# Iselix/kwiiyatta

Measured on AMD Instinct MI355X. Metric: frames/sec end-to-end analyse->align->convert->synth, 48 kHz 5 ms hop, higher is better.
Workload: dtype f64; 1 GPU; config3: 48 kHz source (10 s, T=2001) + target (11 s, T=2201) pairs: CheapTrick+D4C of both, pad with freshly drawn silent spectra, sp2mc, FastDTW(radius 32) align, GMM(64 comp, D=144)+MLPG convert, mc2sp, WORLD synthesis; pairs_per_gpu=32, streams_per_gpu=4, GPU_MAX_HW_QUEUES=4, launch=the whole step is one captured HIP graph, gmm_model_prepared=once per converter (the per-mixture matrices depend on the GMM only), parallelism=pairs in lockstep x32 per GPU, pair-per-GPU x1, no collective

## Files before the change

### kwiiyatta_amd/csrc/kwy_synth.hip

```cpp
#include <math.h>
#include <stdlib.h>

#include <algorithm>
#include <vector>

#include "kwy_internal.hpp"

#define SYN_DEFAULT_F0 500.0
#define SYN_TILE_PER_THREAD 4
#define SYN_TILE (KWY_THREADS * SYN_TILE_PER_THREAD)
#define SYN_TWO_PI (2.0 * KWY_PI)
#define SYN_SLOTS(y_length, fs) ((int)((y_length) * 640 / (fs)) + 64)

struct syn_params {
  int64_t T, y_length;
  int fs, fft_size;
  double frame_period;
  double lowest_f0;
  double sp_mul;
};

__device__ __forceinline__ double syn_increment(const double *__restrict__ f0, const syn_params &p,
                                                int64_t n, double *vuv_out) {
  const double fp = p.frame_period;
// ... 459 lines not shown
          int i = tid * SYN_PH_PER_THREAD + j;
          if (i >= pos && i < cross) {
            if (direct) wrap[tile0 + i] = fmod(ldexp((double)mv[j], k - 52), SYN_TWO_PI);
            if (i == cross - 1) s_tp = ldexp((double)mv[j], k - 52);
          }
        }
        if (cross > pos && !direct) {
          if (tid == 0) { segs[tix].start[nseg] = pos; segs[tix].end[nseg] = cross; segs[tix].tp[nseg] = tp; }
          ++nseg;
        }
        __syncthreads();
        if (cross > pos) tp = s_tp;
      }
      if (cross < tile_n && tp == 0.0) {
        const int nw = min(SYN_WARM, tile_n - cross);
        if (tid < nw) s_c[tid] = inc[tile0 + cross + tid];
        __syncthreads();
        if (tid == 0) {
          double t = 0.0;
          int q = 0;
          for (; q + 8 <= nw; q += 8) {
            double v[8];
#pragma unroll
            for (int u = 0; u < 8; ++u) v[u] = s_c[q + u];
#pragma unroll
            for (int u = 0; u < 8; ++u) { t = t + v[u]; v[u] = t; }
#pragma unroll
            for (int u = 0; u < 8; ++u) s_tps[q + u] = v[u];
          }
          for (; q < nw; ++q) { t = t + s_c[q]; s_tps[q] = t; }
          s_tp = t;
        }
        __syncthreads();
        if (tid < nw) wrap[tile0 + cross + tid] = fmod(s_tps[tid], SYN_TWO_PI);
        tp = s_tp;
        pos = cross + nw;
      } else if (cross < tile_n) {
        tp = tp + inc[tile0 + cross];
        if (tid == 0) wrap[tile0 + cross] = fmod(tp, SYN_TWO_PI);
        pos = cross + 1;
      } else {
        pos = tile_n;
      }
      __syncthreads();
      ++n_rounds;
    }
    if (tid == 0) segs[tix].n = nseg;
    ++tix;
    SYN_DBG_SLOW();
  }
  if (dbg && tid == 0) {
    dbg[40] = clock64() - t_begin; dbg[41] = wall_clock64() - w_begin; dbg[42] = t_fast; dbg[43] = t_slow;
    dbg[44] = n_fast; dbg[45] = n_slow; dbg[46] = n_rounds;
  }
}

__device__ __forceinline__ void syn_tile_apply_body(const double *__restrict__ inc, int64_t y_length,
                                                               const double *__restrict__ tin,
                                                               const syn_segs *__restrict__ segs,
                                                               double *__restrict__ wrap) {
  __shared__ syn_ff wtot[2 * KWY_WAVES + 1];
  const int t = blockIdx.x, tid = threadIdx.x;
  const double tp_tile = tin[t];
  const bool fast = tp_tile > 0.0;
  const int ns = fast ? 1 : segs[t].n;
  const int64_t base = (int64_t)t * SYN_PH_TILE + (int64_t)tid * SYN_TL_PER_THREAD;
  double c[SYN_TL_PER_THREAD];
#pragma unroll
  for (int j = 0; j < SYN_TL_PER_THREAD; ++j) c[j] = (base + j < y_length) ? inc[base + j] : 0.0;
  double tpv[SYN_TL_PER_THREAD];
#pragma unroll
  for (int j = 0; j < SYN_TL_PER_THREAD; ++j) tpv[j] = -1.0;
  for (int q = 0; q < ns; ++q) {
    const double tp = fast ? tp_tile : segs[t].tp[q];
    const int s0 = fast ? 0 : segs[t].start[q], s1 = fast ? SYN_PH_TILE : segs[t].end[q];
    const int k = syn_exponent(tp);
    const unsigned long long tb = (unsigned long long)__double_as_longlong(tp);
    const long long m_in = (long long)((tb & 0xfffffffffffffULL) | 0x10000000000000ULL);
    const bool active = ((tid | 63) + 1) * SYN_TL_PER_THREAD > s0 && (tid & ~63) * SYN_TL_PER_THREAD < s1;
    syn_ff f[SYN_TL_PER_THREAD];
    syn_ff mine = {0, 0};
    if (active) {
#pragma unroll
      for (int j = 0; j < SYN_TL_PER_THREAD; ++j) {
        const int li = tid * SYN_TL_PER_THREAD + j;
        f[j] = (li >= s0 && li < s1 && base + j < y_length) ? syn_ff_make(c[j], k) : syn_ff{0, 0};
        mine = syn_ff_compose(mine, f[j]);
      }
    }
    syn_ff all;
    const syn_ff excl = syn_ff_block_exscan<KWY_WAVES>(mine, wtot, &all);
    if (active) {
      long long m = m_in + ((m_in & 1) ? excl.d1 : excl.d0);
#pragma unroll
      for (int j = 0; j < SYN_TL_PER_THREAD; ++j) {
        const int li = tid * SYN_TL_PER_THREAD + j;
        if (li >= s0 && li < s1 && base + j < y_length) {
          m += (m & 1) ? f[j].d1 : f[j].d0;
          tpv[j] = ldexp((double)m, k - 52);
        }
      }
    }
    __syncthreads();
  }
#pragma unroll
  for (int j = 0; j < SYN_TL_PER_THREAD; ++j)
    if (tpv[j] >= 0.0) wrap[base + j] = fmod(tpv[j], SYN_TWO_PI);
}

__device__ __forceinline__ bool syn_is_pulse(const double *__restrict__ wrap, int64_t n, int64_t y_length) {
  return n < y_length - 1 && fabs(wrap[n + 1] - wrap[n]) > KWY_PI;
}

__device__ __forceinline__ void syn_pulse_count_body(const double *__restrict__ wrap,
                                                                int64_t y_length, int *__restrict__ cnt) {
  __shared__ int sh[KWY_WAVES];
  const int64_t base = (int64_t)blockIdx.x * SYN_TILE + (int64_t)threadIdx.x * SYN_TILE_PER_THREAD;
  int c = 0;
#pragma unroll
  for (int j = 0; j < SYN_TILE_PER_THREAD; ++j) c += syn_is_pulse(wrap, base + j, y_length) ? 1 : 0;
  int tot;
  (void)kwy_block_exscan(c, sh, &tot);
  if (threadIdx.x == 0) cnt[blockIdx.x] = tot;
}

__device__ __forceinline__ void syn_pulse_emit_body(const double *__restrict__ wrap,
                                                               int64_t y_length, int fs,
                                                               const int *__restrict__ tile_off,
                                                               int cap, int32_t *__restrict__ pidx,
                                                               double *__restrict__ pshift) {
  __shared__ int sh[KWY_WAVES];
  const int64_t base = (int64_t)blockIdx.x * SYN_TILE + (int64_t)threadIdx.x * SYN_TILE_PER_THREAD;
  int c = 0;
#pragma unroll
  for (int j = 0; j < SYN_TILE_PER_THREAD; ++j) c += syn_is_pulse(wrap, base + j, y_length) ? 1 : 0;
  int tot;
  int pos = tile_off[blockIdx.x] + kwy_block_exscan(c, sh, &tot);
#pragma unroll
  for (int j = 0; j < SYN_TILE_PER_THREAD; ++j) {
    int64_t n = base + j;
    if (syn_is_pulse(wrap, n, y_length)) {
      if (pos < cap) {
        double y1 = wrap[n] - SYN_TWO_PI;
        double y2 = wrap[n + 1];
        double xx = -y1 / (y2 - y1);
        pidx[pos] = (int32_t)n;
        pshift[pos] = xx / fs;
      }
      ++pos;
    }
  }
}

struct syn_plan {
  int *npulse;
  int *tile_cnt;
  unsigned char *vuv8;
  int32_t *pidx;
  double *pshift;
};
struct syn_plan_view {
  const double *f0;
  syn_params p;
  syn_plan pl;
  double *incr, *wrap, *tsum, *tin;
  long long *summ;
  syn_segs *segs;
  syn_chunks *chunks;
  int cap;
};
struct syn_plan_batch {
  int n;
  long long *dbg;
  syn_plan_view u[KWY_BATCH_MAX];
};
__device__ __forceinline__ int syn_npt(int64_t y_length) { return (int)((y_length + SYN_PH_TILE - 1) / SYN_PH_TILE); }
__device__ __forceinline__ int syn_nt(int64_t y_length) { return (int)((y_length + SYN_TILE - 1) / SYN_TILE); }

__global__ __launch_bounds__(KWY_THREADS) void k_syn_inc(syn_plan_batch b) {
  const syn_plan_view &v = b.u[blockIdx.y];
  syn_inc_body(v.f0, v.p, v.incr, v.pl.vuv8);
}
__global__ __launch_bounds__(KWY_THREADS) void k_syn_tile_sums(syn_plan_batch b) {
  const syn_plan_view &v = b.u[blockIdx.y];
  if ((int)blockIdx.x >= syn_npt(v.p.y_length)) return;
  syn_tile_sums_body(v.incr, v.p.y_length, v.tsum);
}
__global__ __launch_bounds__(KWY_THREADS) void k_syn_tile_summary(syn_plan_batch b) {
  const syn_plan_view &v = b.u[blockIdx.y];
  const int npt = syn_npt(v.p.y_length);
  if ((int)blockIdx.x >= npt) return;
  syn_tile_summary_body(v.incr, v.p.y_length, v.tsum, npt, v.summ, v.chunks);
}
__global__ __launch_bounds__(SYN_PH_THREADS) void k_syn_phase(syn_plan_batch b) {
  const syn_plan_view &v = b.u[blockIdx.x];
  syn_phase_body(v.incr, v.p.y_length, v.summ, v.tin, v.segs, v.chunks, v.wrap, b.dbg);
}
__global__ __launch_bounds__(KWY_THREADS) void k_syn_tile_apply(syn_plan_batch b) {
  const syn_plan_view &v = b.u[blockIdx.y];
  if ((int)blockIdx.x >= syn_npt(v.p.y_length)) return;
  syn_tile_apply_body(v.incr, v.p.y_length, v.tin, v.segs, v.wrap);
}
__global__ __launch_bounds__(KWY_THREADS) void k_syn_pulse_count(syn_plan_batch b) {
  const syn_plan_view &v = b.u[blockIdx.y];
  if ((int)blockIdx.x >= syn_nt(v.p.y_length)) return;
  syn_pulse_count_body(v.wrap, v.p.y_length, v.pl.tile_cnt);
}
__global__ __launch_bounds__(KWY_THREADS) void k_syn_scan_counts(syn_plan_batch b) {
  const syn_plan_view &v = b.u[blockIdx.x];
  syn_scan_counts_body(v.pl.tile_cnt, syn_nt(v.p.y_length), v.pl.npulse);
}
__global__ __launch_bounds__(KWY_THREADS) void k_syn_pulse_emit(syn_plan_batch b) {
  const syn_plan_view &v = b.u[blockIdx.y];
  if ((int)blockIdx.x >= syn_nt(v.p.y_length)) return;
  syn_pulse_emit_body(v.wrap, v.p.y_length, v.p.fs, v.pl.tile_cnt, v.cap, v.pl.pidx, v.pl.pshift);
}

template <int LOG2N>
struct syn_pulse_nt { static constexpr int value = LOG2N <= 10 ? 64 : (LOG2N == 11 ? 128 : 256); };

template <int LOG2N>
struct syn_pulse_form {
  static constexpr bool SHORT = LOG2N == 11;
  static constexpr bool E_IN_BUF = SHORT, HALF_FIRST = SHORT, FUSED_FOLD = SHORT;
  static constexpr int H = 1 << (LOG2N - 1), TWL = (H / 8 > 1) ? H / 8 : 1;
  static constexpr size_t lds = sizeof(kwy_c) * ((H + 1) + TWL) + sizeof(double) * ((H + 2) + 8) +
                                (E_IN_BUF ? 0 : sizeof(uint32_t) * KWY_EBASE_WORDS);
};

template <int LOG2H, int NT, int V>
__device__ inline void syn_rfft_inplace(kwy_c *z, const kwy_c *__restrict__ tw, const kwy_c *__restrict__ pw, const kwy_c (&base)[V],
                                        const kwy_c *__restrict__ twN) {
  kwy_fft_inplace<LOG2H, NT, false>(z, tw, pw);
  kwy_syn_rsplit<LOG2H, NT, V>(z, base, twN);
}

template <int LOG2H, int NT, int V>
__device__ inline void syn_irfft_inplace(kwy_c *z, const kwy_c *__restrict__ tw, const kwy_c *__restrict__ pw, const kwy_c (&base)[V],
                                         const kwy_c *__restrict__ twN) {
  constexpr int H = 1 << LOG2H, N = 2 * H;
  constexpr bool TABLE = 8 * (NT * V) / N < 1;
  const int tid = kwy_tid_opaque();
  __syncthreads();
#pragma unroll
  for (int r = 0; r * NT <= H / 2; ++r) {
    const int k = tid + NT * r;
    if (k > H / 2) continue;
    if (k == 0) {
      const double ar = z[0].x, br = z[H].x;
      z[0] = {ar + br, ar - br};
    } else {
      kwy_c w;
      if constexpr (TABLE) w = twN[k]; else w = syn_pair_twiddle<LOG2H, NT, V>(base, r);
      const kwy_c A = z[k], Bc = z[H - k];
      const double er = A.x + Bc.x, ei = A.y - Bc.y;
      const double dr = A.x - Bc.x, di = A.y + Bc.y;
      const double wr = w.x, wi = -w.y;
      const double orr = __builtin_fma(dr, wr, -(di * wi)), oi = __builtin_fma(dr, wi, di * wr);
      z[k] = {er - oi, ei + orr};
      if (k != H - k) z[H - k] = {er + oi, -(ei - orr)};
    }
  }
  __syncthreads();
  kwy_fft_inplace<LOG2H, NT, true>(z, tw, pw);
}

template <int NT, int V>
__device__ __forceinline__ double syn_block_sum_v(const double (&part)[V], double *red) {
  double ws[V];
#pragma unroll
  for (int g = 0; g < V; ++g) ws[g] = kwy_wave_sum(part[g]);
  __syncthreads();
  if ((threadIdx.x & 63) == 0) {
#pragma unroll
    for (int g = 0; g < V; ++g) red[(threadIdx.x >> 6) + (NT / 64) * g] = ws[g];
  }
  __syncthreads();
  double s = red[0];
#pragma unroll
  for (int i = 1; i < NT * V / 64; ++i) s += red[i];
  return s;
}

__device__ __forceinline__ double syn_safe_ap(double x) {
  return fmax(0.001, fmin(0.999999999999, x));
}

struct syn_view {
  const double *sp, *ap;
  syn_params p;
  const int32_t *pidx;
  const double *pshift;
  const unsigned char *vuv8;
  const int *npulse, *tile_off;
  int cap, slots, nt;
  double *resp, *y;
};
typedef kwy_batch<syn_view> syn_batch;

template <int LOG2N, bool DIRECT>
__global__ __launch_bounds__(syn_pulse_nt<LOG2N>::value, LOG2N <= 11 ? 3 : (LOG2N == 12 ? 2 : 1)) void k_syn_pulse(
    syn_batch batch, kwy_randn_src rs, const uint4 *__restrict__ poly,
    const kwy_c *__restrict__ twH, const kwy_c *__restrict__ twP, const kwy_c *__restrict__ twN,
    const double *__restrict__ dc_remover, long long *__restrict__ dbg) {
  constexpr int NT = syn_pulse_nt<LOG2N>::value, V = KWY_THREADS / NT;
  bool stamping = false;
#define SYN_STAMP(n) do { if (stamping && threadIdx.x == 0) dbg[n] = clock64(); } while (0)
  const int utt = batch.find(blockIdx.x);
  const int lblock = (int)blockIdx.x - batch.start[utt], lgrid = batch.start[utt + 1] - batch.start[utt];
  const double *__restrict__ sp = batch.u[utt].sp, *__restrict__ ap = batch.u[utt].ap;
  const syn_params p = batch.u[utt].p;
  const int32_t *__restrict__ pidx = batch.u[utt].pidx;
  const double *__restrict__ pshift = batch.u[utt].pshift;
  const unsigned char *__restrict__ vuv8 = batch.u[utt].vuv8;
  const int *__restrict__ npulse = batch.u[utt].npulse;
  const int cap = batch.u[utt].cap;
  const int first_pulse = DIRECT ? batch.u[utt].slots : 0, slots = DIRECT ? cap : batch.u[utt].slots;
  double *__restrict__ resp = batch.u[utt].resp;
  double *__restrict__ y = batch.u[utt].y;
  constexpr int N = 1 << LOG2N, H = N / 2, K = H + 1;
  constexpr int C = N / NT;
  constexpr int RK = (H + 1 + NT - 1) / NT;
  constexpr int TWL = (H / 8 > 1) ? H / 8 : 1;
  typedef syn_pulse_form<LOG2N> F;
  extern __shared__ double smem[];
  double *red = smem;
  uint32_t *e_own = (uint32_t *)(red + 8);
  kwy_c *twl = (kwy_c *)(e_own + (F::E_IN_BUF ? 0 : KWY_EBASE_WORDS));
  kwy_c *buf = twl + TWL;
  double *lap = (double *)(buf + (H + 1));
  uint32_t *e = F::E_IN_BUF ? (uint32_t *)(buf + 512) : e_own;
  static_assert(!F::E_IN_BUF || sizeof(kwy_c) * (H + 1) >= 8192 + sizeof(uint32_t) * KWY_EBASE_WORDS, "no room");

  const int tid = threadIdx.x;
  for (int i = tid; i < TWL; i += NT) twl[i] = twH[i];
  kwy_c twb[V];
#pragma unroll
  for (int g = 0; g < V; ++g) twb[g] = twN[tid + NT * g];
  const int P = min(npulse[0], cap);
  const int pend = min(P, first_pulse + slots);
  for (int pp = first_pulse + lblock; pp < pend; pp += lgrid) {
    const int tid = kwy_tid_opaque();
    const int idx = pidx[pp];
    const int nxt = pidx[min(P - 1, pp + 1)];
    const int noise_size = nxt - idx;
    __syncthreads();
    if (noise_size <= 0) continue;
    const int ns_used = min(noise_size, N);
    const double current_vuv = vuv8[idx] ? 1.0 : 0.0;
    const double current_time = idx / (double)p.fs;
    const double shift = pshift[pp];

    int fl = (int)floor(current_time / p.frame_period);
    int ce = (int)ceil(current_time / p.frame_period);
    if (fl > p.T - 1) fl = (int)p.T - 1;
    if (ce > p.T - 1) ce = (int)p.T - 1;
    const double interpolation = current_time / p.frame_period - fl;
    const double *s0 = sp + (int64_t)fl * K, *s1 = sp + (int64_t)ce * K;
    const double *a0 = ap + (int64_t)fl * K, *a1 = ap + (int64_t)ce * K;
    double rv0 = syn_safe_ap(a0[0]);
    if (fl != ce) rv0 = (1.0 - interpolation) * rv0 + interpolation * syn_safe_ap(a1[0]);
    const bool has_periodic = current_vuv > 0.5 && !(rv0 * rv0 > 0.999);
    stamping = dbg && threadIdx.x == 0 && has_periodic && blockIdx.x >= (unsigned)dbg[63] && dbg[62] == 0 &&
               atomicCAS((unsigned long long *)&dbg[62], 0ull, 1ull) == 0ull;
    SYN_STAMP(0);
    {
      double *L = (double *)buf;
      double evs[RK], rts[RK];
#pragma unroll
      for (int r = 0; r < RK; ++r) {
        const int k = min(tid + NT * r, H);
        double ev, rv;
        if (fl == ce) {
          ev = fabs(s0[k] * p.sp_mul);
          rv = syn_safe_ap(a0[k]);
        } else {
          ev = (1.0 - interpolation) * fabs(s0[k] * p.sp_mul) + interpolation * fabs(s1[k] * p.sp_mul);
          rv = (1.0 - interpolation) * syn_safe_ap(a0[k]) + interpolation * syn_safe_ap(a1[k]);
        }
        evs[r] = ev;
        rts[r] = rv * rv;
      }
#pragma unroll
      for (int r = 0; r < RK; ++r) {
        const int k = tid + NT * r;
        if (k <= H) {
          lap[k] = kwy_log((current_vuv != 0.0) ? evs[r] * rts[r] : evs[r]) / 2.0;
          if (has_periodic) L[k] = kwy_log(evs[r] * (1.0 - rts[r]) + KWY_SAFE) / 2.0;
        }
      }
    }

    double dc_component = 0.0;
    SYN_STAMP(1);
#pragma nounroll
    for (int part = has_periodic ? 0 : 1; part < 2; ++part) {
      const int tid = kwy_tid_opaque();
      double *L = (double *)buf;
      if (part == 1) {
        double la[RK], wv[RK];
#pragma unroll
        for (int r = 0; r < RK; ++r) {
          const int k = tid + NT * r;
          la[r] = k <= H ? lap[k] : 0.0;
          wv[r] = (has_periodic && k < H) ? L[k] : 0.0;
        }
        __syncthreads();
#pragma unroll
        for (int r = 0; r < RK; ++r) {
          const int k = tid + NT * r;
          if (k <= H) { L[k] = la[r]; lap[k] = wv[r]; }
        }
      }
      kwy_c mp[RK];
#pragma unroll
      for (int r = 0; r < RK; ++r) mp[r] = {0.0, 0.0};
#pragma nounroll
      for (int it = 0; it < 2 + part; ++it) {
        const int tid = kwy_tid_opaque();
        bool dense_first = true;
        if (it == 0) {
          __syncthreads();
          for (int i = H + 1 + tid; i < N; i += NT) L[i] = L[N - i];
          __syncthreads();
        } else if (it == 1) {
          if constexpr (!F::FUSED_FOLD) kwy_syn_fold<LOG2N - 1, NT, !F::HALF_FIRST>(buf);
          if constexpr (F::HALF_FIRST) {
            kwy_fft_pass8_first_half_core<LOG2N - 1, NT, false>(buf, kwy_tw_table{twl});
            dense_first = false;
          }
        } else {
#pragma unroll
          for (int r = 0; r < RK; ++r) {
            const int k = tid + NT * r;
            mp[r] = k <= H ? buf[k] : kwy_c{0.0, 0.0};
          }
          __syncthreads();
          const uint64_t dpos = (uint64_t)(idx - pidx[0]);
          uint32_t raw[C];
          if (dpos + (uint64_t)ns_used <= rs.n) {
#pragma unroll
            for (int j = 0; j < C; ++j) raw[j] = (tid + NT * j < ns_used) ? rs.tab[dpos + tid + NT * j] : 0u;
          } else {
            kwy_rng_block_ebase(dpos, rs.pow2, e);
            kwy_rng rng;
            if constexpr (sizeof(kwy_c) * (H + 1) >= 8192) {
              kwy_rng_build_table<NT>(e, (uint4 *)buf);
              __syncthreads();
              rng = kwy_rng_combine_table((const uint4 *)buf, poly[tid]);
              __syncthreads();
            } else {
              rng = kwy_rng_combine(e, poly[tid]);
            }
            uint32_t *D = (uint32_t *)buf;
#pragma unroll
            for (int j = 0; j < C; ++j) D[C * tid + j] = kwy_rng_randn_raw(rng);
            __syncthreads();
#pragma unroll
            for (int j = 0; j < C; ++j) raw[j] = D[tid + NT * j];
            __syncthreads();
          }
          double nv[C];
          double sum[V];
#pragma unroll
          for (int g = 0; g < V; ++g) sum[g] = 0.0;
#pragma unroll
          for (int j = 0; j < C; ++j) {
            const int d = tid + NT * j;
            nv[j] = kwy_randn_from_raw(raw[j]);
            if (d < ns_used) sum[j % V] += nv[j];
          }
          const double average = syn_block_sum_v<NT, V>(sum, red) / noise_size;
#pragma unroll
          for (int j = 0; j < C; ++j) {
            const int d = tid + NT * j;
            L[d] = (d < ns_used) ? nv[j] - average : 0.0;
          }
          __syncthreads();
        }
        if constexpr (!F::SHORT) {
          syn_rfft_inplace<LOG2N - 1, NT, V>(buf, twl, twP, twb, twN);
        } else {
          if (dense_first) kwy_fft_pass8<LOG2N - 1, 0, NT, false>(buf, twl);
          kwy_fft_inplace_rest<LOG2N - 1, NT, false>(buf, twl, twP);
          if (F::FUSED_FOLD && it == 0) kwy_syn_rsplit_fold<LOG2N - 1, NT, V, !F::HALF_FIRST>(buf, twb, twN);
          else kwy_syn_rsplit<LOG2N - 1, NT, V>(buf, twb, twN);
        }
        if (it == 1) {
          constexpr int G = 3;
#pragma nounroll
          for (int k0 = tid; k0 <= H; k0 += G * NT) {
            kwy_c R[G];
#pragma unroll
            for (int g = 0; g < G; ++g) R[g] = buf[min(k0 + g * NT, H)];
#pragma unroll
            for (int g = 0; g < G; ++g) {
              const double tmp = exp(R[g].x / N);
              const double ph = R[g].y / N;
              double sn, cs;
              kwy_sincos_medium(ph, &sn, &cs);
              R[g] = {tmp * cs, tmp * sn};
            }
#pragma unroll
            for (int g = 0; g < G; ++g)
              if (k0 + g * NT <= H) buf[k0 + g * NT] = R[g];
          }
          __syncthreads();
        }
      }
      SYN_STAMP(2 + 5 * part);
      if (part == 0) {
        const double coefficient = 2.0 * KWY_PI * shift * p.fs / N;
        for (int k = tid; k <= H; k += NT) {
          const double re = buf[k].x, im = buf[k].y;
          const double re2 = kwy_cos_pi_range(coefficient * k);
          const double im2 = sqrt(1.0 - re2 * re2);
          buf[k] = {__builtin_fma(re, re2, im * im2), __builtin_fma(im, re2, -(re * im2))};
        }
      } else {
#pragma unroll
        for (int r = 0; r < RK; ++r) {
          const int k = tid + NT * r;
          if (k <= H) buf[k] = cmulf(mp[r], buf[k]);
        }
      }
      SYN_STAMP(3 + 5 * part);
      syn_irfft_inplace<LOG2N - 1, NT, V>(buf, twl, twP, twb, twN);
      SYN_STAMP(4 + 5 * part);
      if (part == 0) {
        const double *w = (const double *)buf;
        double ps[V];
#pragma unroll
        for (int g = 0; g < V; ++g) {
          ps[g] = 0.0;
          for (int i = tid + NT * g; i < H; i += KWY_THREADS) ps[g] += w[i];
        }
        dc_component = syn_block_sum_v<NT, V>(ps, red);
        SYN_STAMP(5);
      }
    }
    {
      const int tid = kwy_tid_opaque();
      SYN_STAMP(10);
      const double *w = (const double *)buf;
      const double sqrt_noise_size = sqrt((double)noise_size);
      double *slot = DIRECT ? nullptr : resp + (size_t)(pp - first_pulse) * N;
      const int64_t offset = (int64_t)idx - H + 1;
#pragma unroll
      for (int m = 0; m < C; ++m) {
        int i = tid + NT * m;
        double aper = (i < H) ? w[i + H] : w[i - H];
        double pv = 0.0;
        if (has_periodic) pv = (i < H) ? -dc_component * dc_remover[i] : lap[i - H] - dc_component * dc_remover[i];
        const double r = (pv * sqrt_noise_size + aper) / N;
        if constexpr (DIRECT) {
          const int64_t n = offset + i;
          if (n >= 0 && n < p.y_length) y[n] += r;
        } else {
          slot[i] = r;
        }
      }
      SYN_STAMP(11);
    }
  }
#undef SYN_STAMP
}


#ifndef SYN_OLA_GROUP
#define SYN_OLA_GROUP 4
#endif
__global__ __launch_bounds__(KWY_THREADS) void k_syn_ola(syn_batch batch, int N) {
  const int utt = batch.find(blockIdx.x);
  const double *__restrict__ resp = batch.u[utt].resp;
  const int32_t *__restrict__ pidx = batch.u[utt].pidx;
  const int *__restrict__ tile_off = batch.u[utt].tile_off;
  const int *__restrict__ npulse = batch.u[utt].npulse;
  const int cap = batch.u[utt].cap, nt = batch.u[utt].nt, first_pulse = 0, slots = batch.u[utt].slots;
  const int64_t y_length = batch.u[utt].p.y_length;
  double *__restrict__ y = batch.u[utt].y;
  const int H = N / 2;
  const int tile = (int)blockIdx.x - batch.start[utt];
  const int P = min(npulse[0], cap);
  if (first_pulse >= P && first_pulse > 0) return;
  const int reach = (H + SYN_TILE - 1) / SYN_TILE;
  const int ja = max(0, tile - reach), jb = min(nt - 1, tile + reach);
  int p0 = min(tile_off[ja], P), p1 = jb + 1 < nt ? min(tile_off[jb + 1], P) : P;
  p0 = max(p0, first_pulse);
  p1 = min(p1, first_pulse + slots);
  const int64_t n0 = (int64_t)tile * SYN_TILE + threadIdx.x;
  double v[SYN_TILE_PER_THREAD];
#pragma unroll
  for (int m = 0; m < SYN_TILE_PER_THREAD; ++m) {
    const int64_t n = n0 + KWY_THREADS * m;
    v[m] = (first_pulse > 0 && n < y_length) ? y[n] : 0.0;
  }
  __shared__ int32_t s_idx[KWY_THREADS + 1];
  for (int c0 = p0; c0 < p1; c0 += KWY_THREADS) {
    const int cn = min(KWY_THREADS, p1 - c0);
    __syncthreads();
    if ((int)threadIdx.x < cn) s_idx[threadIdx.x] = pidx[min(P - 1, c0 + (int)threadIdx.x)];
    if (threadIdx.x == 0) s_idx[cn] = pidx[min(P - 1, c0 + cn)];
    __syncthreads();
    for (int g0 = 0; g0 < cn; g0 += SYN_OLA_GROUP) {
      double r[SYN_OLA_GROUP][SYN_TILE_PER_THREAD];
      bool on[SYN_OLA_GROUP][SYN_TILE_PER_THREAD];
#pragma unroll
      for (int g = 0; g < SYN_OLA_GROUP; ++g) {
        const int e = min(g0 + g, cn - 1);
        const int idx = s_idx[e];
        const bool live = g0 + g < cn && s_idx[e + 1] - idx > 0;
        const double *slot = resp + (size_t)(c0 + e - first_pulse) * N;
        const int64_t base = (int64_t)idx - H + 1;
#pragma unroll
        for (int m = 0; m < SYN_TILE_PER_THREAD; ++m) {
          const int64_t q = n0 + KWY_THREADS * m - base;
          on[g][m] = live && q >= 0 && q < N;
          r[g][m] = on[g][m] ? slot[q] : 0.0;
        }
      }
#pragma unroll
      for (int g = 0; g < SYN_OLA_GROUP; ++g) {
#pragma unroll
        for (int m = 0; m < SYN_TILE_PER_THREAD; ++m)
          if (on[g][m]) v[m] += r[g][m];
      }
    }
  }
#pragma unroll
  for (int m = 0; m < SYN_TILE_PER_THREAD; ++m) {
    const int64_t n = n0 + KWY_THREADS * m;
    if (n < y_length) y[n] = v[m];
  }
}

static int get_dc_remover(kwy_ctx *ctx, int fft_size, const double **out) {
  std::string key = "dcrem:" + std::to_string(fft_size);
  return kwy_cached_table<double>(ctx, key, [&] {
    std::vector<double> h(fft_size);
    double dc_component = 0.0;
    for (int i = 0; i < fft_size / 2; ++i) {
      h[i] = 0.5 - 0.5 * cos(2.0 * KWY_PI * (i + 1.0) / (1.0 + fft_size));
      h[fft_size - i - 1] = h[i];
      dc_component += h[i] * 2.0;
    }
    for (int i = 0; i < fft_size / 2; ++i) {
      h[i] /= dc_component;
      h[fft_size - i - 1] = h[i];
    }
    return h;
  }, out);
}

template <int LOG2N>
static int launch_pulse(kwy_ctx *ctx, syn_batch &batch) {
  constexpr int N = 1 << LOG2N, H = N / 2, K = H + 1;
  const kwy_c *twH, *twN, *twP;
  const uint4 *poly;
  const double *dcrem;
  KWY_TRY(kwy_get_twiddles(ctx, LOG2N - 1, &twH));
  KWY_TRY(kwy_get_twiddle_powers(ctx, LOG2N - 1, &twP));
  KWY_TRY(kwy_get_twiddles(ctx, LOG2N, &twN));
  KWY_TRY(kwy_get_poly(ctx, 12ull * (N / syn_pulse_nt<LOG2N>::value), &poly));
  KWY_TRY(get_dc_remover(ctx, N, &dcrem));
  constexpr int NT = syn_pulse_nt<LOG2N>::value;
  static_assert(K + 1 == syn_pulse_form<LOG2N>::H + 2, "the log-spectrum rows");
  size_t lds = syn_pulse_form<LOG2N>::lds;
  KWY_HIP(hipFuncSetAttribute((const void *)k_syn_pulse<LOG2N, false>,
                              hipFuncAttributeMaxDynamicSharedMemorySize, (int)lds));
  KWY_HIP(hipFuncSetAttribute((const void *)k_syn_pulse<LOG2N, true>,
                              hipFuncAttributeMaxDynamicSharedMemorySize, (int)lds));
  const int share = batch.n > 1 ? std::max(64, 4096 / batch.n) : 2048;
  int g = 0;
  for (int u = 0; u < batch.n; ++u) { batch.start[u] = g; g += std::max(1, std::min(batch.u[u].slots, share)); }
  batch.start[batch.n] = g;
  KWY_PROF(ctx, "k_syn_pulse", hipLaunchKernelGGL((k_syn_pulse<LOG2N, false>), dim3(g), dim3(NT), lds, ctx->stream, batch,
                     kwy_randn(ctx), poly, twH, twP, twN, dcrem, (long long *)ctx->dbg));
  g = 0;
  for (int u = 0; u < batch.n; ++u) { batch.start[u] = g; g += batch.u[u].nt; }
  batch.start[batch.n] = g;
  KWY_PROF(ctx, "k_syn_ola", hipLaunchKernelGGL(k_syn_ola, dim3(g), dim3(KWY_THREADS), 0, ctx->stream, batch, N));
  for (int u = 0; u <= batch.n; ++u) batch.start[u] = u;
  KWY_PROF(ctx, "k_syn_pulse_more", hipLaunchKernelGGL((k_syn_pulse<LOG2N, true>), dim3(batch.n), dim3(NT), lds, ctx->stream,
                     batch, kwy_randn(ctx), poly, twH, twP, twN, dcrem, (long long *)nullptr));
  KWY_HIP(hipGetLastError());
  return KWY_OK;
}

static int syn_pulse_cap(int64_t y_length) { return (int)(y_length / 8 + 16); }

static size_t syn_plan_bytes(int64_t y_length);
static size_t syn_plan_scratch_bytes(int64_t y_length);
static size_t syn_render_scratch_bytes(int64_t y_length, int fft_size, int fs) {
  return kwy_pad(sizeof(double) * (size_t)SYN_SLOTS(y_length, fs) * fft_size) + kwy_pad(64);
}
static size_t syn_scratch_bytes(int64_t y_length, int fft_size, int fs) {
  return syn_plan_bytes(y_length) + syn_plan_scratch_bytes(y_length) + syn_render_scratch_bytes(y_length, fft_size, fs);
}

static size_t syn_plan_bytes(int64_t y_length) {
  const int64_t nt = (y_length + SYN_TILE - 1) / SYN_TILE;
  const int cap = syn_pulse_cap(y_length);
  return kwy_pad(64) + kwy_pad(sizeof(int) * (nt + 1)) + kwy_pad(y_length) + kwy_pad(sizeof(int32_t) * cap) +
         kwy_pad(sizeof(double) * cap);
}

static syn_plan syn_plan_carve(void *buffer, int64_t y_length) {
  const int64_t nt = (y_length + SYN_TILE - 1) / SYN_TILE;
  const int cap = syn_pulse_cap(y_length);
  char *q = (char *)buffer;
  syn_plan pl;
  pl.npulse = (int *)q; q += kwy_pad(64);
  pl.tile_cnt = (int *)q; q += kwy_pad(sizeof(int) * (nt + 1));
  pl.vuv8 = (unsigned char *)q; q += kwy_pad(y_length);
  pl.pidx = (int32_t *)q; q += kwy_pad(sizeof(int32_t) * cap);
  pl.pshift = (double *)q;
  return pl;
}

static int syn_make_params(kwy_ctx *ctx, int64_t T, int fft_size, double frame_period_ms, int fs, double sp_mul,
                           int64_t y_length, syn_params *p, int *log2n) {
  *log2n = kwy_ilog2(fft_size);
  if ((1 << *log2n) != fft_size || *log2n < 9 || *log2n > 13) {
    ctx->err = "synthesize: fft_size must be a power of two in [512, 8192]";
    return KWY_EINVAL;
  }
  p->T = T; p->y_length = y_length; p->fs = fs; p->fft_size = fft_size;
  p->frame_period = frame_period_ms / 1000.0;
  p->lowest_f0 = fs / fft_size + 1.0;
  p->sp_mul = sp_mul;
  return KWY_OK;
}

static size_t syn_plan_scratch_bytes(int64_t y_length) {
  return 2 * kwy_pad(sizeof(double) * y_length) + 5 * kwy_pad(8 * (y_length / 4096 + 2)) + kwy_pad(64) +
         kwy_pad(sizeof(syn_segs) * (y_length / 4096 + 2)) + kwy_pad(sizeof(syn_chunks) * (y_length / 4096 + 2));
}

static int syn_plan_fill(kwy_ctx *ctx, const double *f0, const syn_params &p, const syn_plan &pl, syn_plan_view *v) {
  const int64_t y_length = p.y_length;
  const size_t npt_alloc = (size_t)((y_length + SYN_PH_TILE - 1) / SYN_PH_TILE) + 1;
  v->f0 = f0; v->p = p; v->pl = pl;
  v->cap = syn_pulse_cap(y_length);
  v->incr = kwy_arena<double>(ctx, y_length);
  v->tsum = kwy_arena<double>(ctx, npt_alloc);
  v->tin = kwy_arena<double>(ctx, npt_alloc);
  v->summ = kwy_arena<long long>(ctx, 3 * npt_alloc);
  v->segs = kwy_arena<syn_segs>(ctx, npt_alloc);
  v->chunks = kwy_arena<syn_chunks>(ctx, npt_alloc);
  v->wrap = kwy_arena<double>(ctx, y_length);
  if (!v->incr || !v->tsum || !v->tin || !v->summ || !v->segs || !v->chunks || !v->wrap) {
    ctx->err = "synthesize: scratch arena too small";
    return KWY_ENOMEM;
  }
  return KWY_OK;
}

static int synth_plan_launch(kwy_ctx *ctx, syn_plan_batch &b) {
  int64_t ymax = 0;
  for (int u = 0; u < b.n; ++u) ymax = std::max(ymax, b.u[u].p.y_length);
  for (int u = b.n; u < KWY_BATCH_MAX; ++u) b.u[u] = b.u[0];
  b.dbg = (long long *)ctx->dbg;
  const unsigned n = (unsigned)b.n;
  const unsigned npt = (unsigned)((ymax + SYN_PH_TILE - 1) / SYN_PH_TILE), nt = (unsigned)((ymax + SYN_TILE - 1) / SYN_TILE);
  hipLaunchKernelGGL(k_syn_inc, dim3((unsigned)((ymax + KWY_THREADS - 1) / KWY_THREADS), n), dim3(KWY_THREADS), 0,
                     ctx->stream, b);
  hipLaunchKernelGGL(k_syn_tile_sums, dim3(npt, n), dim3(KWY_THREADS), 0, ctx->stream, b);
  hipLaunchKernelGGL(k_syn_tile_summary, dim3(npt, n), dim3(KWY_THREADS), 0, ctx->stream, b);
  KWY_PROF(ctx, "k_syn_phase", hipLaunchKernelGGL(k_syn_phase, dim3(n), dim3(SYN_PH_THREADS), 0, ctx->stream, b));
  hipLaunchKernelGGL(k_syn_tile_apply, dim3(npt, n), dim3(KWY_THREADS), 0, ctx->stream, b);
  hipLaunchKernelGGL(k_syn_pulse_count, dim3(nt, n), dim3(KWY_THREADS), 0, ctx->stream, b);
  hipLaunchKernelGGL(k_syn_scan_counts, dim3(n), dim3(KWY_THREADS), 0, ctx->stream, b);
  hipLaunchKernelGGL(k_syn_pulse_emit, dim3(nt, n), dim3(KWY_THREADS), 0, ctx->stream, b);
  KWY_HIP(hipGetLastError());
  return KWY_OK;
}

static int synth_plan(kwy_ctx *ctx, const double *f0, const syn_params &p, const syn_plan &pl) {
  syn_plan_batch b;
  b.n = 1;
  KWY_TRY(syn_plan_fill(ctx, f0, p, pl, &b.u[0]));
  return synth_plan_launch(ctx, b);
}

static int syn_fill_view(kwy_ctx *ctx, const syn_plan &pl, const double *sp, const double *ap, const syn_params &p,
                         double *y, syn_view *v) {
  const int64_t y_length = p.y_length;
  v->sp = sp; v->ap = ap; v->p = p;
  v->pidx = pl.pidx; v->pshift = pl.pshift; v->vuv8 = pl.vuv8; v->npulse = pl.npulse; v->tile_off = pl.tile_cnt;
  v->cap = syn_pulse_cap(y_length);
  v->slots = SYN_SLOTS(y_length, p.fs);
  v->nt = (int)((y_length + SYN_TILE - 1) / SYN_TILE);
  v->resp = kwy_arena<double>(ctx, (size_t)v->slots * p.fft_size);
  v->y = y;
  if (!v->resp) { ctx->err = "synthesize: scratch arena too small"; return KWY_ENOMEM; }
  return KWY_OK;
}

static int syn_launch(kwy_ctx *ctx, syn_batch &batch, int log2n) {
  switch (log2n) {
    case 9: return launch_pulse<9>(ctx, batch);
    case 10: return launch_pulse<10>(ctx, batch);
    case 11: return launch_pulse<11>(ctx, batch);
    case 12: return launch_pulse<12>(ctx, batch);
    default: return launch_pulse<13>(ctx, batch);
  }
}

static int synth_render(kwy_ctx *ctx, const syn_plan &pl, const double *sp, const double *ap, const syn_params &p,
                        int log2n, double *y) {
  syn_batch batch;
  batch.n = 1;
  KWY_TRY(syn_fill_view(ctx, pl, sp, ap, p, y, &batch.u[0]));
  return syn_launch(ctx, batch, log2n);
}

static int synth_core(kwy_ctx *ctx, const double *f0, int64_t T, const double *sp, const double *ap,
                      int fft_size, double frame_period_ms, int fs, double sp_mul, int64_t y_length,
                      double *y) {
  syn_params p;
  int log2n;
  KWY_TRY(syn_make_params(ctx, T, fft_size, frame_period_ms, fs, sp_mul, y_length, &p, &log2n));
  if (y_length < 2 || T < 2) {
    KWY_HIP(hipMemsetAsync(y, 0, sizeof(double) * y_length, ctx->stream));
    return KWY_OK;
  }
  void *buffer = kwy_arena_alloc(ctx, syn_plan_bytes(y_length));
  if (!buffer) { ctx->err = "synthesize: scratch arena too small"; return KWY_ENOMEM; }
  const syn_plan pl = syn_plan_carve(buffer, y_length);
  KWY_TRY(synth_plan(ctx, f0, p, pl));
  return synth_render(ctx, pl, sp, ap, p, log2n, y);
}

static int syn_check(kwy_ctx *ctx, const void *f0, int64_t T, const void *sp, const void *ap,
                     int fft_size, double frame_period_ms, int fs, int64_t y_length, const void *y) {
  if (!ctx) return KWY_EINVAL;
  if (!f0 || !sp || !ap || !y || T <= 0 || fs <= 0 || fft_size <= 0 || !(frame_period_ms > 0) ||
      y_length < 0 || y_length > 0x7fffffff) {
    ctx->err = "synthesize: bad argument";
    return KWY_EINVAL;
  }
  return KWY_OK;
}

extern "C" int kwy_synthesize_dev(kwy_ctx *ctx, const double *f0, int64_t T, const double *sp,
                                  const double *ap, int fft_size, double frame_period_ms, int fs,
                                  double sp_mul, int64_t y_length, double *y) {
  KWY_TRY(syn_check(ctx, f0, T, sp, ap, fft_size, frame_period_ms, fs, y_length, y));
  KWY_HIP(hipSetDevice(ctx->device));
  if (y_length == 0) return KWY_OK;
  KWY_TRY(kwy_arena_begin(ctx, syn_scratch_bytes(y_length, fft_size, fs)));
  return synth_core(ctx, f0, T, sp, ap, fft_size, frame_period_ms, fs, sp_mul, y_length, y);
}

extern "C" int64_t kwy_synth_plan_bytes(int64_t y_length) {
  return y_length >= 0 && y_length <= 0x7fffffff ? (int64_t)syn_plan_bytes(y_length) : 0;
}

extern "C" int kwy_synth_plan_dev(kwy_ctx *ctx, const double *f0, int64_t T, int fft_size, double frame_period_ms,
                                  int fs, int64_t y_length, void *plan) {
  KWY_TRY(syn_check(ctx, f0, T, f0, f0, fft_size, frame_period_ms, fs, y_length, f0));
  if (!plan) { ctx->err = "synth_plan: bad argument"; return KWY_EINVAL; }
  KWY_HIP(hipSetDevice(ctx->device));
  syn_params p;
  int log2n;
  KWY_TRY(syn_make_params(ctx, T, fft_size, frame_period_ms, fs, 1.0, y_length, &p, &log2n));
  if (y_length < 2 || T < 2) return KWY_OK;
  KWY_TRY(kwy_arena_begin(ctx, syn_plan_scratch_bytes(y_length)));
  return synth_plan(ctx, f0, p, syn_plan_carve(plan, y_length));
}

extern "C" int kwy_synth_plan_batch_dev(kwy_ctx *ctx, const kwy_synth_plan_job *jobs, int count, int fft_size,
                                        double frame_period_ms, int fs) {
  if (!ctx) return KWY_EINVAL;
  if (!jobs || count < 0) { ctx->err = "synth_plan_batch: bad argument"; return KWY_EINVAL; }
  KWY_HIP(hipSetDevice(ctx->device));
  size_t bytes = 0;
  for (int j = 0; j < count; ++j) {
    const kwy_synth_plan_job &q = jobs[j];
    KWY_TRY(syn_check(ctx, q.f0, q.f0_length, q.f0, q.f0, fft_size, frame_period_ms, fs, q.y_length, q.f0));
    if (!q.plan) { ctx->err = "synth_plan_batch: bad argument"; return KWY_EINVAL; }
    bytes += syn_plan_scratch_bytes(q.y_length);
  }
  KWY_TRY(kwy_arena_begin(ctx, bytes));
  syn_plan_batch b;
  b.n = 0;
  for (int j = 0; j < count; ++j) {
    const kwy_synth_plan_job &q = jobs[j];
    syn_params p;
    int log2n;
    KWY_TRY(syn_make_params(ctx, q.f0_length, fft_size, frame_period_ms, fs, 1.0, q.y_length, &p, &log2n));
    if (q.y_length < 2 || q.f0_length < 2) continue;
    KWY_TRY(syn_plan_fill(ctx, q.f0, p, syn_plan_carve(q.plan, q.y_length), &b.u[b.n]));
    if (++b.n == KWY_BATCH_MAX) { KWY_TRY(synth_plan_launch(ctx, b)); b.n = 0; }
  }
  if (b.n > 0) KWY_TRY(synth_plan_launch(ctx, b));
  return KWY_OK;
}

extern "C" int kwy_synth_render_dev(kwy_ctx *ctx, const void *plan, int64_t T, const double *sp, const double *ap,
                                    int fft_size, double frame_period_ms, int fs, double sp_mul, int64_t y_length,
                                    double *y) {
  KWY_TRY(syn_check(ctx, sp, T, sp, ap, fft_size, frame_period_ms, fs, y_length, y));
  if (!plan) { ctx->err = "synth_render: bad argument"; return KWY_EINVAL; }
  KWY_HIP(hipSetDevice(ctx->device));
  if (y_length == 0) return KWY_OK;
  syn_params p;
  int log2n;
  KWY_TRY(syn_make_params(ctx, T, fft_size, frame_period_ms, fs, sp_mul, y_length, &p, &log2n));
  if (y_length < 2 || T < 2) {
    KWY_HIP(hipMemsetAsync(y, 0, sizeof(double) * y_length, ctx->stream));
    return KWY_OK;
  }
  KWY_TRY(kwy_arena_begin(ctx, syn_render_scratch_bytes(y_length, fft_size, fs)));
  return synth_render(ctx, syn_plan_carve(const_cast<void *>(plan), y_length), sp, ap, p, log2n, y);
}

#define SYN_RENDER_GROUP 4
extern "C" int kwy_synth_render_batch_dev(kwy_ctx *ctx, const kwy_synth_job *jobs, int count, int fft_size,
                                          double frame_period_ms, int fs, double sp_mul) {
  if (!ctx) return KWY_EINVAL;
  if (!jobs || count < 0) { ctx->err = "synth_render_batch: bad argument"; return KWY_EINVAL; }
  KWY_HIP(hipSetDevice(ctx->device));
  size_t bytes = 0, group = 0;
  int in_group = 0;
  for (int j = 0; j < count; ++j) {
    const kwy_synth_job &q = jobs[j];
    KWY_TRY(syn_check(ctx, q.spectrogram, q.f0_length, q.spectrogram, q.aperiodicity, fft_size, frame_period_ms, fs,
                      q.y_length, q.y));
    if (!q.plan) { ctx->err = "synth_render_batch: bad argument"; return KWY_EINVAL; }
    if (q.y_length < 2 || q.f0_length < 2) continue;
    group += syn_render_scratch_bytes(q.y_length, fft_size, fs);
    if (++in_group == SYN_RENDER_GROUP) { bytes = std::max(bytes, group); group = 0; in_group = 0; }
  }
  bytes = std::max(bytes, group);
  KWY_TRY(kwy_arena_begin(ctx, bytes));
  syn_batch batch;
  batch.n = 0;
  int log2n = 0;
  for (int j = 0; j < count; ++j) {
    const kwy_synth_job &q = jobs[j];
    if (q.y_length == 0) continue;
    syn_params p;
    KWY_TRY(syn_make_params(ctx, q.f0_length, fft_size, frame_period_ms, fs, sp_mul, q.y_length, &p, &log2n));
    if (q.y_length < 2 || q.f0_length < 2) {
      KWY_HIP(hipMemsetAsync(q.y, 0, sizeof(double) * q.y_length, ctx->stream));
      continue;
    }
    KWY_TRY(syn_fill_view(ctx, syn_plan_carve(const_cast<void *>(q.plan), q.y_length), q.spectrogram, q.aperiodicity, p,
                          q.y, &batch.u[batch.n]));
    if (++batch.n == SYN_RENDER_GROUP) {
      KWY_TRY(syn_launch(ctx, batch, log2n));
      batch.n = 0;
      ctx->arena_off = 0;
    }
  }
  if (batch.n > 0) KWY_TRY(syn_launch(ctx, batch, log2n));
  return KWY_OK;
}

extern "C" int kwy_synthesize(kwy_ctx *ctx, const double *f0, int64_t T, const double *sp,
                              const double *ap, int fft_size, double frame_period_ms, int fs,
                              double sp_mul, int64_t y_length, double *y) {
  KWY_TRY(syn_check(ctx, f0, T, sp, ap, fft_size, frame_period_ms, fs, y_length, y));
  KWY_HIP(hipSetDevice(ctx->device));
  if (y_length == 0) return KWY_OK;
  for (int64_t i = 0; i < T; ++i)
    if (!(f0[i] >= 0.0 && f0[i] < fs / 12.0)) { ctx->err = "synthesize: f0 must lie in [0, fs/12)"; return KWY_EINVAL; }
  const int K = fft_size / 2 + 1;
  kwy_staging st(ctx, "synthesize");
  double *df0, *dsp, *dap, *dy;
  st.in(df0, f0, (size_t)T);
  st.in(dsp, sp, (size_t)T * K);
  st.in(dap, ap, (size_t)T * K);
  st.out(dy, y, (size_t)y_length);
  KWY_TRY(st.begin(syn_scratch_bytes(y_length, fft_size, fs)));
  KWY_TRY(synth_core(ctx, df0, T, dsp, dap, fft_size, frame_period_ms, fs, sp_mul, y_length, dy));
  return st.finish();
}
```

Measured before the change: 2.929 million frames/s.

## Use persistent ticket-based pulse scheduling and larger synth render groups

Replaces the static per-utterance block partition of the pulse kernel with a persistent grid sized to resident occupancy. Blocks pull pulse indices from a global atomic ticket counter across all utterances in the batch, and the next ticket is prefetched in double-buffered shared memory. The render group is raised from 4 to the batch maximum, so more utterances share one launch sequence. Short outputs are now zeroed with a small kernel instead of hipMemsetAsync. The change targets load imbalance and launch count, at the cost of an atomic per pulse and a head-reset kernel per pass.

```diff
diff --git a/kwiiyatta_amd/csrc/kwy_synth.hip b/kwiiyatta_amd/csrc/kwy_synth.hip
--- a/kwiiyatta_amd/csrc/kwy_synth.hip
+++ b/kwiiyatta_amd/csrc/kwy_synth.hip
@@ -785,22 +785,21 @@
 __global__ __launch_bounds__(syn_pulse_nt<LOG2N>::value, LOG2N <= 11 ? 3 : (LOG2N == 12 ? 2 : 1)) void k_syn_pulse(
     syn_batch batch, kwy_randn_src rs, const uint4 *__restrict__ poly,
     const kwy_c *__restrict__ twH, const kwy_c *__restrict__ twP, const kwy_c *__restrict__ twN,
-    const double *__restrict__ dc_remover, long long *__restrict__ dbg) {
+    const double *__restrict__ dc_remover, unsigned *__restrict__ head, long long *__restrict__ dbg) {
   constexpr int NT = syn_pulse_nt<LOG2N>::value, V = KWY_THREADS / NT;
   bool stamping = false;
 #define SYN_STAMP(n) do { if (stamping && threadIdx.x == 0) dbg[n] = clock64(); } while (0)
-  const int utt = batch.find(blockIdx.x);
-  const int lblock = (int)blockIdx.x - batch.start[utt], lgrid = batch.start[utt + 1] - batch.start[utt];
+  int utt = DIRECT ? (int)blockIdx.x : 0, base = 0;
   const double *__restrict__ sp = batch.u[utt].sp, *__restrict__ ap = batch.u[utt].ap;
-  const syn_params p = batch.u[utt].p;
+  syn_params p = batch.u[utt].p;
   const int32_t *__restrict__ pidx = batch.u[utt].pidx;
   const double *__restrict__ pshift = batch.u[utt].pshift;
   const unsigned char *__restrict__ vuv8 = batch.u[utt].vuv8;
-  const int *__restrict__ npulse = batch.u[utt].npulse;
-  const int cap = batch.u[utt].cap;
-  const int first_pulse = DIRECT ? batch.u[utt].slots : 0, slots = DIRECT ? cap : batch.u[utt].slots;
+  const int first_pulse = DIRECT ? batch.u[utt].slots : 0;
   double *__restrict__ resp = batch.u[utt].resp;
   double *__restrict__ y = batch.u[utt].y;
+  int P = min(batch.u[utt].npulse[0], batch.u[utt].cap);
+  int end = DIRECT ? P : min(P, batch.u[utt].slots);
   constexpr int N = 1 << LOG2N, H = N / 2, K = H + 1;
   constexpr int C = N / NT;
   constexpr int RK = (H + 1 + NT - 1) / NT;
@@ -820,14 +819,34 @@
   kwy_c twb[V];
 #pragma unroll
   for (int g = 0; g < V; ++g) twb[g] = twN[tid + NT * g];
-  const int P = min(npulse[0], cap);
-  const int pend = min(P, first_pulse + slots);
-  for (int pp = first_pulse + lblock; pp < pend; pp += lgrid) {
+  static_assert(KWY_THREADS / 64 <= 4, "the block sums use red[0 .. 4), the tickets live in red[4]");
+  int *tick = (int *)(red + 4);
+  if constexpr (!DIRECT) {
+    if (tid == 0) tick[0] = (int)atomicAdd(head, 1u);
+  }
+  for (int pp = first_pulse - 1, par = 1;;) {
     const int tid = kwy_tid_opaque();
+    if constexpr (DIRECT) {
+      if (++pp >= end) return;
+    } else {
+      par ^= 1;
+      __syncthreads();
+      const int ticket = __builtin_amdgcn_readfirstlane(tick[par]);
+      while (ticket >= end) {
+        if (++utt >= batch.n) return;
+        sp = batch.u[utt].sp; ap = batch.u[utt].ap; p = batch.u[utt].p;
+        pidx = batch.u[utt].pidx; pshift = batch.u[utt].pshift; vuv8 = batch.u[utt].vuv8; resp = batch.u[utt].resp;
+        P = min(batch.u[utt].npulse[0], batch.u[utt].cap);
+        base = end;
+        end += min(P, batch.u[utt].slots);
+      }
+      pp = ticket - base;
+      if (tid == 0) tick[par ^ 1] = (int)atomicAdd(head, 1u);
+    }
     const int idx = pidx[pp];
     const int nxt = pidx[min(P - 1, pp + 1)];
     const int noise_size = nxt - idx;
-    __syncthreads();
+    if constexpr (DIRECT) __syncthreads();
     if (noise_size <= 0) continue;
     const int ns_used = min(noise_size, N);
     const double current_vuv = vuv8[idx] ? 1.0 : 0.0;
@@ -1117,6 +1136,12 @@
   }
 }
 
+__global__ __launch_bounds__(KWY_THREADS) void k_syn_zero(double *__restrict__ y, int64_t n, unsigned *__restrict__ head) {
+  const int64_t i = (int64_t)blockIdx.x * KWY_THREADS + threadIdx.x;
+  if (i < n) y[i] = 0.0;
+  if (head && i == 0) *head = 0u;
+}
+
 static int get_dc_remover(kwy_ctx *ctx, int fft_size, const double **out) {
   std::string key = "dcrem:" + std::to_string(fft_size);
   return kwy_cached_table<double>(ctx, key, [&] {
@@ -1136,7 +1161,7 @@
 }
 
 template <int LOG2N>
-static int launch_pulse(kwy_ctx *ctx, syn_batch &batch) {
+static int launch_pulse(kwy_ctx *ctx, syn_batch &batch, unsigned *head) {
   constexpr int N = 1 << LOG2N, H = N / 2, K = H + 1;
   const kwy_c *twH, *twN, *twP;
   const uint4 *poly;
@@ -1153,19 +1178,25 @@
                               hipFuncAttributeMaxDynamicSharedMemorySize, (int)lds));
   KWY_HIP(hipFuncSetAttribute((const void *)k_syn_pulse<LOG2N, true>,
                               hipFuncAttributeMaxDynamicSharedMemorySize, (int)lds));
-  const int share = batch.n > 1 ? std::max(64, 4096 / batch.n) : 2048;
-  int g = 0;
-  for (int u = 0; u < batch.n; ++u) { batch.start[u] = g; g += std::max(1, std::min(batch.u[u].slots, share)); }
-  batch.start[batch.n] = g;
+  int64_t &resident = ctx->i_vals[std::string("syn_resident_") + std::to_string(LOG2N)];
+  if (!resident) {
+    int cus = 0, per_cu = 0;
+    KWY_HIP(hipDeviceGetAttribute(&cus, hipDeviceAttributeMultiprocessorCount, ctx->device));
+    KWY_HIP(hipOccupancyMaxActiveBlocksPerMultiprocessor(&per_cu, (const void *)k_syn_pulse<LOG2N, false>, NT, lds));
+    resident = (int64_t)std::max(1, cus) * std::max(1, per_cu);
+  }
+  int64_t most = 0;
+  for (int u = 0; u < batch.n; ++u) most += std::min(batch.u[u].slots, batch.u[u].cap);
+  int g = (int)std::max<int64_t>(1, std::min(most, resident));
+  hipLaunchKernelGGL(k_syn_zero, dim3(1), dim3(KWY_THREADS), 0, ctx->stream, (double *)nullptr, (int64_t)0, head);
   KWY_PROF(ctx, "k_syn_pulse", hipLaunchKernelGGL((k_syn_pulse<LOG2N, false>), dim3(g), dim3(NT), lds, ctx->stream, batch,
-                     kwy_randn(ctx), poly, twH, twP, twN, dcrem, (long long *)ctx->dbg));
+                     kwy_randn(ctx), poly, twH, twP, twN, dcrem, head, (long long *)ctx->dbg));
   g = 0;
   for (int u = 0; u < batch.n; ++u) { batch.start[u] = g; g += batch.u[u].nt; }
   batch.start[batch.n] = g;
   KWY_PROF(ctx, "k_syn_ola", hipLaunchKernelGGL(k_syn_ola, dim3(g), dim3(KWY_THREADS), 0, ctx->stream, batch, N));
-  for (int u = 0; u <= batch.n; ++u) batch.start[u] = u;
   KWY_PROF(ctx, "k_syn_pulse_more", hipLaunchKernelGGL((k_syn_pulse<LOG2N, true>), dim3(batch.n), dim3(NT), lds, ctx->stream,
-                     batch, kwy_randn(ctx), poly, twH, twP, twN, dcrem, (long long *)nullptr));
+                     batch, kwy_randn(ctx), poly, twH, twP, twN, dcrem, (unsigned *)nullptr, (long long *)nullptr));
   KWY_HIP(hipGetLastError());
   return KWY_OK;
 }
@@ -1174,8 +1205,12 @@
 
 static size_t syn_plan_bytes(int64_t y_length);
 static size_t syn_plan_scratch_bytes(int64_t y_length);
+static size_t syn_slot_bytes(int64_t y_length, int fft_size, int fs) {
+  return kwy_pad(sizeof(double) * (size_t)SYN_SLOTS(y_length, fs) * fft_size);
+}
+static size_t syn_head_bytes() { return kwy_pad(sizeof(unsigned)); }
 static size_t syn_render_scratch_bytes(int64_t y_length, int fft_size, int fs) {
-  return kwy_pad(sizeof(double) * (size_t)SYN_SLOTS(y_length, fs) * fft_size) + kwy_pad(64);
+  return syn_slot_bytes(y_length, fft_size, fs) + syn_head_bytes();
 }
 static size_t syn_scratch_bytes(int64_t y_length, int fft_size, int fs) {
   return syn_plan_bytes(y_length) + syn_plan_scratch_bytes(y_length) + syn_render_scratch_bytes(y_length, fft_size, fs);
@@ -1280,13 +1315,13 @@
   return KWY_OK;
 }
 
-static int syn_launch(kwy_ctx *ctx, syn_batch &batch, int log2n) {
+static int syn_launch(kwy_ctx *ctx, syn_batch &batch, int log2n, unsigned *head) {
   switch (log2n) {
-    case 9: return launch_pulse<9>(ctx, batch);
-    case 10: return launch_pulse<10>(ctx, batch);
-    case 11: return launch_pulse<11>(ctx, batch);
-    case 12: return launch_pulse<12>(ctx, batch);
-    default: return launch_pulse<13>(ctx, batch);
+    case 9: return launch_pulse<9>(ctx, batch, head);
+    case 10: return launch_pulse<10>(ctx, batch, head);
+    case 11: return launch_pulse<11>(ctx, batch, head);
+    case 12: return launch_pulse<12>(ctx, batch, head);
+    default: return launch_pulse<13>(ctx, batch, head);
   }
 }
 
@@ -1294,8 +1329,10 @@
                         int log2n, double *y) {
   syn_batch batch;
   batch.n = 1;
+  unsigned *head = kwy_arena<unsigned>(ctx, 1);
+  if (!head) { ctx->err = "synthesize: scratch arena too small"; return KWY_ENOMEM; }
   KWY_TRY(syn_fill_view(ctx, pl, sp, ap, p, y, &batch.u[0]));
-  return syn_launch(ctx, batch, log2n);
+  return syn_launch(ctx, batch, log2n, head);
 }
 
 static int synth_core(kwy_ctx *ctx, const double *f0, int64_t T, const double *sp, const double *ap,
@@ -1399,7 +1436,10 @@
   return synth_render(ctx, syn_plan_carve(const_cast<void *>(plan), y_length), sp, ap, p, log2n, y);
 }
 
-#define SYN_RENDER_GROUP 4
+#ifndef SYN_RENDER_GROUP
+#define SYN_RENDER_GROUP KWY_BATCH_MAX
+#endif
+static_assert(SYN_RENDER_GROUP >= 1 && SYN_RENDER_GROUP <= KWY_BATCH_MAX, "a pass is one job table");
 extern "C" int kwy_synth_render_batch_dev(kwy_ctx *ctx, const kwy_synth_job *jobs, int count, int fft_size,
                                           double frame_period_ms, int fs, double sp_mul) {
   if (!ctx) return KWY_EINVAL;
@@ -1413,11 +1453,14 @@
                       q.y_length, q.y));
     if (!q.plan) { ctx->err = "synth_render_batch: bad argument"; return KWY_EINVAL; }
     if (q.y_length < 2 || q.f0_length < 2) continue;
-    group += syn_render_scratch_bytes(q.y_length, fft_size, fs);
+    group += syn_slot_bytes(q.y_length, fft_size, fs);
     if (++in_group == SYN_RENDER_GROUP) { bytes = std::max(bytes, group); group = 0; in_group = 0; }
   }
   bytes = std::max(bytes, group);
-  KWY_TRY(kwy_arena_begin(ctx, bytes));
+  KWY_TRY(kwy_arena_begin(ctx, syn_head_bytes() + bytes));
+  unsigned *head = kwy_arena<unsigned>(ctx, 1);
+  if (!head) { ctx->err = "synth_render_batch: scratch arena too small"; return KWY_ENOMEM; }
+  const size_t pool = ctx->arena_off;
   syn_batch batch;
   batch.n = 0;
   int log2n = 0;
@@ -1427,18 +1470,20 @@
     syn_params p;
     KWY_TRY(syn_make_params(ctx, q.f0_length, fft_size, frame_period_ms, fs, sp_mul, q.y_length, &p, &log2n));
     if (q.y_length < 2 || q.f0_length < 2) {
-      KWY_HIP(hipMemsetAsync(q.y, 0, sizeof(double) * q.y_length, ctx->stream));
+      hipLaunchKernelGGL(k_syn_zero, dim3((unsigned)((q.y_length + KWY_THREADS - 1) / KWY_THREADS)), dim3(KWY_THREADS), 0,
+                         ctx->stream, q.y, (int64_t)q.y_length, (unsigned *)nullptr);
+      KWY_HIP(hipGetLastError());
       continue;
     }
     KWY_TRY(syn_fill_view(ctx, syn_plan_carve(const_cast<void *>(q.plan), q.y_length), q.spectrogram, q.aperiodicity, p,
                           q.y, &batch.u[batch.n]));
     if (++batch.n == SYN_RENDER_GROUP) {
-      KWY_TRY(syn_launch(ctx, batch, log2n));
+      KWY_TRY(syn_launch(ctx, batch, log2n, head));
       batch.n = 0;
-      ctx->arena_off = 0;
-    }
-  }
-  if (batch.n > 0) KWY_TRY(syn_launch(ctx, batch, log2n));
+      ctx->arena_off = pool;
+    }
+  }
+  if (batch.n > 0) KWY_TRY(syn_launch(ctx, batch, log2n, head));
   return KWY_OK;
 }
 
```

Result: faster. 2.961 million frames/s (median of 6 runs) (+1.1%).
